# dotchen/LAV

Measured on AMD Instinct MI355X. Metric: frames/s full agent fwd (32k-pt LiDAR + 3 cams), higher is better.
Workload: dtype f32 (convolution contractions on the matrix cores with f32 accumulate at the error of an fp32 dot product, DESIGN 4.3: the layers on the split-operand kernel - BEV backbone, heads, crop stems, the brake net's mid-size layers - and ERFNet's persistent runs of pairs as two power-of-two-scaled fp16 pie

## Files before the change

### include/lav_amd.h

```cpp
#ifndef LAV_AMD_H
#define LAV_AMD_H

#include <stddef.h>
#include <stdint.h>

#ifdef __cplusplus
extern "C" {
#endif

#define LAV_ABI_VERSION 30

#define LAV_OK 0
#define LAV_EINVAL (-1)
#define LAV_EHIP (-2)
#define LAV_EWORKSPACE (-3)

int lav_abi_version(void);
const char *lav_last_error(void);
int lav_device_count(void);

int lav_profile_enable(int slots);
int lav_profile_reset(void);
int lav_profile_read(const char *kernel, double *total_ms, int *launches);

typedef struct lav_grid {
    float min_x, max_x, min_y, max_y;
    float ppm;
    int nx, ny;
} lav_grid;

typedef struct lav_pointnet {
    const float *w1, *b1, *w2, *b2;
    int num_input;
// ... 187 lines not shown

size_t lav_upconv_pointwise_packed_floats(int cin, int cout, int k);
int lav_upconv_pointwise_pack(int cin, int cout, int k, const float *h_weight, float *h_packed);
int lav_upconv_pointwise_parts(int batch, int cin, int cout, int ih, int iw, int k, int pad, int out_pad);
int lav_upconv_pointwise(int batch, int cin, int cout, int ih, int iw, int k, int pad, int out_pad, const float *x, const float *w_packed,
                         const float *scale, const float *shift, int relu_pre, int out_c_total, int out_c_offset, float *y,
                         float *amax_out, void *stream);

size_t lav_conv1d_pair_packed_weight_floats(int channels);
int lav_conv1d_pair_pack_weights(int channels, const float *h_weight, float *h_packed);
size_t lav_conv1d_pair_chain_workspace_bytes(int batch, int h);
size_t lav_conv1d_pair_chain_lds_bytes(int channels, int w, int d_b_max);
int lav_conv1d_pair_chain(int batch, int channels, int h, int w, int npairs, const int *d_a, const int *d_b, const int *residual,
                          const int *relu_post, const float *x, const float *const *wa_packed, const float *const *bias_a,
                          const float *const *wb_packed, const float *const *bias_b, const float *const *scale,
                          const float *const *shift, float *const *out, void *workspace, size_t workspace_bytes, void *stream);
int lav_conv1d_pair_chain_f16(int batch, int channels, int h, int w, int npairs, const int *d_a, const int *d_b, const int *residual,
                              const int *relu_post, const float *x, const float *const *wa_packed, const float *const *bias_a,
                              const float *const *wb_packed, const float *const *bias_b, const float *const *scale,
                              const float *const *shift, float *const *out, void *workspace, size_t workspace_bytes, void *stream);
int lav_conv1d_pair_chain_region(int row_offset, int clean_rows);
int lav_conv1d_pair_chain_status(const void *workspace, int *h_timeouts_launches2, void *stream);
size_t lav_conv1d_pair_lds_bytes(int channels, int w, int d_b);
int lav_conv1d_pair(int batch, int channels, int h, int w, int d_a, int d_b, const float *x, const float *wa_packed,
                    const float *bias_a, const float *wb_packed, const float *bias_b, const float *scale, const float *shift,
                    const float *residual, int relu_post, float *y, void *stream);

int lav_pool_affine(const float *x, int batch, int channels, int h, int w, const float *scale, const float *shift, int relu,
                    float *y, int out_c_total, int out_c_offset, void *stream);

int lav_pair_train_supported(int channels, int width);
size_t lav_pair_train_workspace_bytes(int batch, int channels, int h);
int lav_pair_train_forward(const float *x, const float *wa, const float *ba, const float *wb, const float *bb, int batch, int channels,
                           int h, int w, int dil, float *t, float *z, void *stream);
int lav_pair_train_backward(const float *x, const float *t, const float *dz, const float *wa, const float *wb, int batch, int channels,
                            int h, int w, int dil, float *dt, float *dx, float *dwa, float *dba, float *dwb, float *dbb, void *workspace,
                            size_t workspace_bytes, void *stream);

size_t lav_seg_xent_workspace_bytes(void);
int lav_seg_xent_forward(const float *logits, const long long *labels, int batch, int classes, long plane, float *loss, float *dlogits,
                         void *workspace, size_t workspace_bytes, void *stream);

int lav_seg_xent_up_forward(const float *logits, const void *labels, int label_bytes, int batch, int classes, int h, int w, int scale,
                            float *loss, float *dlogits, void *workspace, size_t workspace_bytes, void *stream);

#ifdef __cplusplus
// ... 4 lines not shown
```

### lav_amd/_lib.py

```python
from __future__ import annotations

import ctypes as C
import os

HERE = os.path.dirname(os.path.abspath(__file__))
LIB_PATH = os.environ.get("LAV_AMD_LIB") or os.path.join(HERE, "liblav_amd.so")

ABI_VERSION = 30
MAX_CAM = 4


class Grid(C.Structure):
    _fields_ = [("min_x", C.c_float), ("max_x", C.c_float), ("min_y", C.c_float), ("max_y", C.c_float),
                ("ppm", C.c_float), ("nx", C.c_int), ("ny", C.c_int)]


class PointNet(C.Structure):
    _fields_ = [("w1", C.c_void_p), ("b1", C.c_void_p), ("w2", C.c_void_p), ("b2", C.c_void_p),
                ("num_input", C.c_int), ("channels", C.c_int)]


class Camera(C.Structure):
    _fields_ = [("K", C.c_float * 9), ("l2w", C.c_float * 16), ("w2c", C.c_float * 16)]


class Conv(C.Structure):
    _fields_ = [(n, C.c_int) for n in (
        "batch", "in_c_total", "in_c_offset", "cin", "h", "w", "cout", "kh", "kw", "stride", "pad_h", "pad_w",
        "dil_h", "dil_w", "transposed", "out_pad", "out_c_total", "out_c_offset", "relu_pre", "relu_post", "sigmoid", "target_cus")] + [("pad_value", C.c_float), ("precision", C.c_int)]


# ... 42 lines not shown
    "lav_conv2d": (_I, [C.POINTER(Conv), _P, _P, _P, _P, _P, _P, _P, _P, _Z, _P]),
    "lav_conv_amax_count": (_I, [C.POINTER(Conv)]),
    "lav_conv2d_amax": (_I, [C.POINTER(Conv), _P, _P, _P, _P, _P, _P, _P, _P, _Z, _P, _I, _P, _P]),
    "lav_deconv_grouped": (_I, [_I, _I, _I, _I, _I, C.POINTER(_I), _I, _I, _I, _I, _P, _P, _P, _I, _P, _P]),
    "lav_crop_rotate": (_I, [_P, _I, _I, _I, _I, _P, _P, _I, _F, _I, _F, _F, _P, _P]),
    "lav_crop_rotate_indexed": (_I, [_P, _I, _P, _I, _I, _I, _P, _P, _I, _F, _I, _F, _F, _P, _P]),
    "lav_crop_rotate_backward": (_I, [_P, _I, _P, _I, _I, _I, _P, _P, _I, _F, _I, _F, _F, _P, _P]),
    "lav_pillar_decorate": (_I, [_P, C.POINTER(_I), _I, _I, _I, C.POINTER(Grid), _P, _P, _P, _P, _P, _P, _Z, _P]),
    "lav_scatter_max": (_I, [_P, _P, _I, _I, _I, _P, _P, _P]),
    "lav_scatter_max_backward": (_I, [_P, _P, _I, _I, _I, _P, _P]),
    "lav_conv1d_pair_packed_weight_floats": (_Z, [_I]),
    "lav_conv1d_pair_pack_weights": (_I, [_I, _P, _P]),
    "lav_upconv_pointwise_packed_floats": (_Z, [_I, _I, _I]),
    "lav_upconv_pointwise_pack": (_I, [_I, _I, _I, _P, _P]),
    "lav_upconv_pointwise_parts": (_I, [_I] * 8),
    "lav_upconv_pointwise": (_I, [_I] * 8 + [_P, _P, _P, _P, _I, _I, _I, _P, _P, _P]),
    "lav_conv1d_pair_chain_workspace_bytes": (_Z, [_I, _I]),
    "lav_conv1d_pair_chain_region": (_I, [_I, _I]),
    "lav_conv1d_pair_chain_lds_bytes": (_Z, [_I, _I, _I]),
    "lav_conv1d_pair_chain": (_I, [_I, _I, _I, _I, _I, C.POINTER(_I), C.POINTER(_I), C.POINTER(_I), C.POINTER(_I), _P] + [C.POINTER(_P)] * 7 + [_P, _Z, _P]),
    "lav_conv1d_pair_chain_f16": (_I, [_I, _I, _I, _I, _I, C.POINTER(_I), C.POINTER(_I), C.POINTER(_I), C.POINTER(_I), _P] + [C.POINTER(_P)] * 7 + [_P, _Z, _P]),
    "lav_conv1d_pair_chain_status": (_I, [_P, C.POINTER(_I), _P]),
    "lav_conv1d_pair_lds_bytes": (_Z, [_I, _I, _I]),
    "lav_conv1d_pair": (_I, [_I, _I, _I, _I, _I, _I, _P, _P, _P, _P, _P, _P, _P, _P, _I, _P, _P]),
    "lav_gru_seq_forward": (_I, [_P, _I, _P, _P, _P, _I, _I, _I, _P, _P, _P]),
    "lav_gru_seq_backward_workspace_bytes": (_Z, [_I, _I]),
    "lav_gru_seq_backward": (_I, [_P, _P, _P, _P, _P, _I, _I, _I, _P, _P, _P, _P, _Z, _P]),
    "lav_bn_train_workspace_bytes": (_Z, [_I]),
    "lav_bn_train_forward_mask": (_I, [_P, _P, _P, _P, _I, _I, C.c_long, _P, _P, C.c_double, _I, _P, _P, _P, _P, _P, _Z, _P]),
    "lav_bn_train_backward_mask": (_I, [_P, _P, _P, _P, _I, _I, C.c_long, _P, _P, _P, _I, _P, _P, _P, _P, _P, _P, _Z, _P]),
    "lav_pair_train_supported": (_I, [_I, _I]),
    "lav_pair_train_workspace_bytes": (_Z, [_I, _I, _I]),
    "lav_pair_train_forward": (_I, [_P, _P, _P, _P, _P, _I, _I, _I, _I, _I, _P, _P, _P]),
    "lav_pair_train_backward": (_I, [_P, _P, _P, _P, _P, _I, _I, _I, _I, _I, _P, _P, _P, _P, _P, _P, _P, _Z, _P]),
    "lav_seg_xent_workspace_bytes": (_Z, []),
    "lav_seg_xent_forward": (_I, [_P, _P, _I, _I, C.c_long, _P, _P, _P, _Z, _P]),
    "lav_seg_xent_up_forward": (_I, [_P, _P, _I, _I, _I, _I, _I, _I, _P, _P, _P, _Z, _P]),
    "lav_attn_train_workspace_bytes": (_Z, [_I, _I, _I, _I]),
    "lav_attn_train_forward": (_I, [_P, _I, _I, _I, _I, _P, _P, _P, _P, C.c_float, _P, _P, _P, _P, _P, _P]),
    "lav_attn_train_backward": (_I, [_P, _I, _I, _I, _I, _P, _P, _P, _P, C.c_float, _P, _P, _P, _P, _P, _P, _P, _P, _P, _Z, _P]),
    "lav_bn_train_forward": (_I, [_P, _P, _P, _I, _I, C.c_long, _P, _P, C.c_double, _I, _I, _P, _P, _P, _P, _Z, _P]),
    "lav_bn_train_backward": (_I, [_P, _P, _P, _I, _I, C.c_long, _P, _P, _P, _I, _I, _P, _P, _P, _P, _P, _Z, _P]),
    "lav_bn_train_amax_count": (_I, [_I, _I, C.c_long]),
    "lav_bn_train_forward_amax": (_I, [_P, _P, _P, _I, _I, C.c_long, _P, _P, C.c_double, _I, _I, _P, _P, _P, _P, _P, _Z, _P]),
    "lav_bn_train_backward_amax": (_I, [_P, _P, _P, _I, _I, C.c_long, _P, _P, _P, _I, _I, _P, _P, _P, _P, _P, _P, _Z, _P]),
    "lav_attn_pool": (_I, [_P, _I, _I, _I, _I, _P, _P, _P, _P, _P, _P]),
# ... 53 lines not shown
```

### lav_amd/build.py

```python
from __future__ import annotations

import os
import subprocess
import sys
import time

HERE = os.path.dirname(os.path.abspath(__file__))
REPO = os.path.dirname(HERE)
CSRC = os.path.join(HERE, "csrc")
LIB = os.path.join(HERE, "liblav_amd.so")
SOURCES = ["misc.hip", "pillar.hip", "paint.hip", "gru.hip", "gru_seq.hip", "conv.hip", "conv_f16.hip", "conv_pair.hip", "deconv.hip", "crop.hip", "frame.hip", "attn.hip", "bn_train.hip", "conv_wgrad.hip", "upconv.hip", "conv_pair_train.hip"]
EXTRA_FLAGS = {"pillar.hip": ["-ffp-contract=off"], "paint.hip": ["-ffp-contract=off"], "crop.hip": ["-ffp-contract=off"],
               "frame.hip": ["-ffp-contract=off"]}
FLAGS = ["--offload-arch=gfx950", "-O3", "-std=c++17", "-fPIC", "-Wall", "-Wno-unused-function", "-fno-slp-vectorize",
         "-I", os.path.join(REPO, "include"), "-I", CSRC]


def _hipcc() -> str:
    for c in (os.environ.get("HIPCC"), "/opt/rocm/bin/hipcc", "hipcc"):
        if c and (os.path.isabs(c) and os.path.exists(c) or not os.path.isabs(c)):
            return c
    raise RuntimeError("hipcc not found")


def needs_build() -> bool:
    if not os.path.exists(LIB):
        return True
    t = os.path.getmtime(LIB)
    deps = [os.path.join(CSRC, f) for f in os.listdir(CSRC)] + [os.path.join(REPO, "include", "lav_amd.h")]
    return any(os.path.getmtime(d) > t for d in deps)


def build(force: bool = False, verbose: bool = True) -> str:
    if not force and not needs_build():
# ... 28 lines not shown
```

### lav_amd/csrc/conv.hip

```cpp
#include <algorithm>
#include <cstdlib>
#include <cstring>
#include <vector>

#include "common.hpp"
#include "conv_f16.hpp"

namespace {
using namespace lav;
typedef float f32x16 __attribute__((ext_vector_type(16)));

constexpr int MAX_TAPS = 64;
constexpr int MAX_CLASSES = 16;
constexpr int CK = 16;
constexpr int TAP_GROUP = 9;
constexpr int NPOS_MAX = 40;

struct ConvArgs {
    const float *x, *w, *bias, *scale, *shift, *res;
    const int *n_valid;
    unsigned long long *trace;
    float *y;
    int in_c_total, in_c_offset, cin, H, W;
    int cout, out_c_total, out_c_offset, OH, OW;
// ... 824 lines not shown
}
}

extern "C" int lav_conv_out_hw(const lav_conv *c, int *oh, int *ow) {
    LAV_REQUIRE(c, "lav_conv_out_hw: null");
    Plan p;
    int rc = build_plan(*c, p);
    if (rc) return rc;
    if (oh) *oh = p.OH;
    if (ow) *ow = p.OW;
    return LAV_OK;
}

extern "C" size_t lav_conv_packed_weight_floats(const lav_conv *c) {
    if (!c) return 0;
    Plan p;
    if (build_plan(*c, p)) return 0;
    const int prec = resolve_precision(*c);
    size_t n = has_split_packing(prec) ? (p.wfloats + 3) / 4 * 4 + split_weight_bytes(p) / 4 : p.wfloats;
    if (prec == LAV_CONV_F16X3 && f16x3_layer(*c, p)) n += split_weight_bytes_f16(p) / 4 + 4;
    return n;
}

extern "C" int lav_conv_pack_weights(const lav_conv *c, const float *h_weight, float *h_packed) {
    LAV_REQUIRE(c && h_weight && h_packed, "lav_conv_pack_weights: null");
    Plan p;
    int rc = build_plan(*c, p);
    if (rc) return rc;
    memset(h_packed, 0, p.wfloats * sizeof(float));
    for (int cls = 0; cls < p.nclasses; ++cls) {
        float *dst = h_packed + p.woff[cls];
        const auto &t = p.taps[cls];
        parallel_for((int)t.size(), [&, dst](int ti_) {
            const size_t ti = (size_t)ti_;
            for (int ci = 0; ci < c->cin; ++ci)
                for (int co = 0; co < c->cout; ++co) {
                    const size_t src = c->transposed
                                           ? (((size_t)ci * c->cout + co) * c->kh + t[ti].ky) * c->kw + t[ti].kx
                                           : (((size_t)co * c->cin + ci) * c->kh + t[ti].ky) * c->kw + t[ti].kx;
                    dst[(size_t)(co / 32) * t.size() * p.cin_pad * 32 + ((ti * p.cin_pad + ci) / 8) * 256 + ((ci & 1) * 32 + co % 32) * 4 + (ci % 8) / 2] = h_weight[src];
                }
        });
    }
    if (has_split_packing(resolve_precision(*c)))
        split_pack_weights(*c, p, h_weight, reinterpret_cast<unsigned char *>(h_packed + (p.wfloats + 3) / 4 * 4));
    if (resolve_precision(*c) == LAV_CONV_F16X3 && f16x3_layer(*c, p))
// ... 339 lines not shown
```

### lav_amd/frame.py

```python
from __future__ import annotations

import math
import os
import time
from collections import deque

import numpy as np
import torch

from . import ops
from .model_inference import InferModel

GAP = 5
_COPY_STREAM = os.environ.get("LAV_COPY_STREAM", "0") == "1"
_DET_REPORT = os.environ.get("LAV_DET_REPORT", "1") != "0"
_POSE_BLOCK = os.environ.get("LAV_POSE_BLOCK", "1") != "0"
_BRAKE_AFTER = os.environ.get("LAV_BRAKE_AFTER", "in")
_BRAKE_SPLIT = os.environ.get("LAV_BRAKE_SPLIT", "wide")
if _BRAKE_SPLIT in ("0", "off", "none"):
    _BRAKE_SPLIT = ""
_DIAG_SKIP = set(filter(None, os.environ.get("LAV_DIAG_SKIP", "").split(",")))


def ego_box_mask(lidar: torch.Tensor) -> torch.Tensor:
# ... 458 lines not shown
                       crop_size=up.crop_size * 2, cmd=int(cmd_value), impl="steps")[0, -1, 0]
        self.plan_aborts += 1
        return plan

    @torch.no_grad()
    @_at_frame_precision
    def plan_deviation(self, out, cmd_value) -> float:
        up = self.infer_model.uniplanner
        with torch.cuda.stream(self.s_ego):
            self.s_ego.wait_stream(torch.cuda.current_stream())
            ego_cast = up.cast(out["ego_embd"], mode="ego")
            plan = up.plan(out["ego_embd"], self.b_nxp[None], cast_locs=ego_cast, pixels_per_meter=up.pixels_per_meter,
                           crop_size=up.crop_size * 2, cmd=int(cmd_value), impl="steps")[0, -1, 0]
            dev = (plan - out["ego_plan_locs"]).abs().max()
        torch.cuda.current_stream().wait_stream(self.s_ego)
        return float(dev)

    def health(self, cmd_value: int = 3) -> dict:
        torch.cuda.synchronize()
        up = self.infer_model.uniplanner
        diag = ops.gru_plan_diag(1, up.plan_gru.hidden_size, up.num_cmds, int(cmd_value), self.device, stream=self.s_ego)
        nonfinite, checks = (int(v) for v in self.d_health.cpu())
        chain_timeouts, chain_launches = ops.pair_chain_status(self.device, stream=self.s_cap)
        nonfinite += self.nonfinite_det_frames
        return dict(nonfinite_outputs=nonfinite, finite_checks=checks, plan_launches=diag["launches"], plan_aborts=diag["aborted_launches"],
                    pair_chain_launches=chain_launches, pair_chain_timeouts=chain_timeouts,
                    plans_recomputed=self.plan_aborts, decode_mismatches=self.decode_mismatches, overflow_ticks=self.overflow_ticks,
                    last_plan_launch=diag)

    @torch.no_grad()
    @_at_frame_precision
    def precapture(self, cmds=range(6), max_others=15):
        dev, P = self.device, self.P
        tick = torch.zeros((P, 4), dtype=torch.float32, device=dev)
        tick[:, 0] = torch.linspace(5.0, 60.0, P, device=dev); tick[:, 2] = -1.0
        rgb = lambda *shape: torch.zeros(shape, dtype=torch.float32, device=dev)
        args = (rgb(3, 3, 288, 256), rgb(1, 3, 288, 768), rgb(1, 3, 192, 480), np.zeros(2), 0.0, torch.zeros(2, device=dev))
        self.step(tick, *args, 3)
        self.step(tick, *args, 3)
        for cmd in cmds:
            with torch.cuda.stream(self.s_ego):
                self._replay(("ego", int(cmd)), self._g_ego, self.s_ego, int(cmd))
        if self.device_others:
            self._replay("others_cap", self._g_others_cap, self.s_cap)
        else:
            for n in range(1, max_others + 1):
                self._replay(("others", n), self._g_others, self.s_cap, n)
        torch.cuda.synchronize()
        self.reset()
# ... 4 lines not shown
```

### lav_amd/lidar.py

```python
from __future__ import annotations

import torch
from torch import nn
import torch.nn.functional as F

from . import _lib
from . import ops
from .ops import Amax, ConvLayer, GroupedDeconv, PointwiseUpconv
from .point_pillar import PointPillarNet

_NORM = dict(eps=1e-3, momentum=0.01)


def _refreshable(obj):
    if isinstance(obj, dict):
        for v in obj.values():
            yield from _refreshable(v)
    elif isinstance(obj, (list, tuple)):
        for v in obj:
            yield from _refreshable(v)
    elif hasattr(obj, "refresh"):
        yield obj


class _Engine(nn.Module):

    def _drop(self):
        object.__setattr__(self, "_eng", None)
        object.__setattr__(self, "_stale", False)

    def _mark_stale(self):
# ... 69 lines not shown
        eng = self._fresh(device) or dict(device=device)
        key = ("backbone", prec)
        if key in eng:
            return eng[key]
        def stage(seq):
            out = []
            for j in range(0, len(seq), 3):
                conv, bn = seq[j], seq[j + 2]
                out.append(ConvLayer(conv.weight, stride=conv.stride[0], padding=conv.padding, bn=_bn_tuple(bn),
                                     bn_eps=bn.eps, relu_pre=True, precision=prec, device=device))
            return out
        ups = []
        off = 0
        for seq in (self.upconv1, self.upconv2, self.upconv3):
            ct, bn = seq[0], seq[2]
            if prec == _lib.CONV_F16X3 and PointwiseUpconv.takes(ct):
                ups.append(PointwiseUpconv(ct, bn, relu_pre=True, out_c_total=self.out_channels, out_c_offset=off, device=device))
            else:
                ups.append(ConvLayer(ct.weight, stride=ct.stride[0], padding=ct.padding, transposed=True,
                                     output_padding=ct.output_padding[0], bn=_bn_tuple(bn), bn_eps=bn.eps, relu_pre=True,
                                     out_c_total=self.out_channels, out_c_offset=off, precision=prec, device=device))
            off += ct.weight.shape[1]
        eng[key] = dict(s1=stage(self.conv1), s2=stage(self.conv2), s3=stage(self.conv3), ups=ups, amax={}, f16=prec == _lib.CONV_F16X3)
        eng["tensor_ids"] = self._tensor_ids()
        object.__setattr__(self, "_eng", eng)
        return eng[key]

    def forward_train(self, x):
        from .train.hipnn import conv_relu_bn
        f1 = conv_relu_bn(self.conv1, x)
        f2 = conv_relu_bn(self.conv2, f1)
        f3 = conv_relu_bn(self.conv3, f2)
        return torch.cat([conv_relu_bn(self.upconv1, f1), conv_relu_bn(self.upconv2, f2), conv_relu_bn(self.upconv3, f3)], dim=1)

    def forward(self, x, out=None):
        if self.training:
            return self.forward_train(x)
        self._need_eval()
        e = self._engine(x.device)
        if not e["f16"]:
            feats = []
            for st in (e["s1"], e["s2"], e["s3"]):
                for layer in st:
                    x = layer(x)
                feats.append(x)
            oh, ow = e["ups"][0].out_hw(feats[0].shape[2], feats[0].shape[3])
            if out is None:
                out = torch.empty((x.shape[0], self.out_channels, oh, ow), dtype=torch.float32, device=x.device)
            for up, f in zip(e["ups"], feats):
                up(f, out=out)
            return out
        B = x.shape[0]
        key = ops.amax_key(x)
        ams = e["amax"].get(key)
        if ams is None:
            ams = e["amax"][key] = [Amax(x.device) for _ in range(len(e["s1"]) + len(e["s2"]) + len(e["s3"]) + 1)]
        stages = (e["s1"], e["s2"], e["s3"])
        feats, feat_am, am_prev, i = [], [], ops.amax_of(x), 0
        for si, st in enumerate(stages):
            for li, layer in enumerate(st):
                oh, ow = layer.out_hw(x.shape[2], x.shape[3])
                readers = ([st[li + 1]] if li + 1 < len(st) else ([stages[si + 1][0]] if si + 1 < len(stages) else [])) + \
                          ([e["ups"][si]] if li + 1 == len(st) else [])
                am = ams[i].reset() if any(r.uses_amax(B, oh, ow) for r in readers) else None
                x = layer(x, amax_in=am_prev, amax_out=am)
                am_prev, i = am, i + 1
            feats.append(x); feat_am.append(am_prev)
        oh, ow = e["ups"][0].out_hw(feats[0].shape[2], feats[0].shape[3])
        if out is None:
            out = torch.empty((B, self.out_channels, oh, ow), dtype=torch.float32, device=x.device)
        am_out = ams[-1].reset()
        for up, f, am in zip(e["ups"], feats, feat_am):
            up(f, out=out, amax_in=am, amax_out=am_out)
        return ops.tag_amax(out, am_out)


class Head(_Engine):
    def __init__(self, num_input, num_output, num_hidden=64, norm_cfg=None, output_activation=nn.Identity()):
        super().__init__()
        self.net = nn.Sequential(
            nn.Conv2d(num_input, num_hidden, 3, 1, 1, bias=False),
            nn.ReLU(inplace=True),
            nn.BatchNorm2d(num_hidden, **_NORM),
            nn.ConvTranspose2d(num_hidden, num_output, 3, 2, 1, 1),
        )
        self.output_activation = output_activation
        self._drop()

    @property
# ... 93 lines not shown
```

### lav_amd/ops.py

```python
from __future__ import annotations

import ctypes as C
import os as _os
import threading as _threading
from typing import Optional, Sequence

import numpy as np
import torch

from . import _lib
from ._lib import Camera, Conv, Grid, PointNet, check

_workspaces: dict = {}


def _stream() -> int:
    return torch.cuda.current_stream().cuda_stream


def _ptr(t: Optional[torch.Tensor]) -> Optional[int]:
    return None if t is None else t.data_ptr()


def _f32c(t: torch.Tensor, name: str) -> torch.Tensor:
# ... 743 lines not shown

    def __enter__(self):
        check(_lib.load().lav_conv1d_pair_chain_region(*self.args), "lav_conv1d_pair_chain_region")
        return self

    def __exit__(self, *exc):
        check(_lib.load().lav_conv1d_pair_chain_region(0, -1), "lav_conv1d_pair_chain_region")
        return False


def pair_chain_status(device, stream=None):
    st = stream if stream is not None else torch.cuda.current_stream()
    device = torch.device(device)
    if device.index is None:
        device = torch.device("cuda", torch.cuda.current_device())
    ws = _workspaces.get(("pair_chain", device, st.cuda_stream))
    if ws is None:
        return (0, 0)
    v = (C.c_int * 2)()
    check(_lib.load().lav_conv1d_pair_chain_status(_ptr(ws), v, st.cuda_stream), "lav_conv1d_pair_chain_status")
    return (int(v[0]), int(v[1]))


_CU_COUNT = {}


def _cu_count(device) -> int:
    idx = torch.device(device).index
    idx = torch.cuda.current_device() if idx is None else idx
    if idx not in _CU_COUNT:
        _CU_COUNT[idx] = torch.cuda.get_device_properties(idx).multi_processor_count
    return _CU_COUNT[idx]


train_work = {"crop_rotate_backward_bytes": 0, "crop_rotate_backward_calls": 0, "gru_seq_forward_flops": 0, "gru_seq_backward_flops": 0,
              "bn_train_fwd_bytes": 0, "bn_train_bwd_bytes": 0, "conv_wgrad_flops": 0}


class _CropRotateIndexed(torch.autograd.Function):

    @staticmethod
    def forward(ctx, features, map_index, locs, oris, ppm, crop, ox, oy):
        lib = _lib.load()
        features = _f32c(features, "features")
        locs, oris = _f32c(locs.detach().reshape(-1, 2), "locs"), _f32c(oris.detach().reshape(-1), "oris")
        if map_index.dtype != torch.int32 or not map_index.is_cuda:
# ... 218 lines not shown
```

Measured before the change: 508.0.

## Fuse BEV backbone stage conv3x3 layers into one persistent fp16-split run kernel

Adds a persistent kernel that runs a stage's sequence of identical 3x3 conv + ReLU + BatchNorm layers in one launch. Blocks own output rows and wait on per-row readiness words from the previous layer instead of relaunching. It applies to the BEV backbone stages s2 and s3 by default, cutting per-layer launch overhead and letting weight prefetch overlap across layers. In exchange it relies on inter-block spin-waiting with a timeout and NaN-fill fallback, and adds ping-pong intermediate buffers.

```diff
diff --git a/include/lav_amd.h b/include/lav_amd.h
--- a/include/lav_amd.h
+++ b/include/lav_amd.h
@@ -8,7 +8,7 @@
 extern "C" {
 #endif
 
-#define LAV_ABI_VERSION 30
+#define LAV_ABI_VERSION 31
 
 #define LAV_OK 0
 #define LAV_EINVAL (-1)
@@ -242,6 +242,15 @@
 int lav_conv1d_pair_chain_region(int row_offset, int clean_rows);
 int lav_conv1d_pair_chain_status(const void *workspace, int *h_timeouts_launches2, void *stream);
 size_t lav_conv1d_pair_lds_bytes(int channels, int w, int d_b);
+size_t lav_conv3x3_run_f16_workspace_bytes(int channels, int h, int w, int nlayers);
+size_t lav_conv3x3_run_f16_lds_bytes(int channels, int h, int w);
+size_t lav_conv3x3_run_f16_weight_bytes(int channels);
+int lav_conv3x3_run_f16_amax_count(int channels, int h, int w);
+long lav_conv_f16_weights_offset(const lav_conv *c);
+int lav_conv3x3_run_f16(int channels, int h, int w, int nlayers, const float *x, const void *const *w_f16, const float *const *scale,
+                        const float *const *shift, float *out, const float *amax_in, int amax_in_count, float *amax_out, void *workspace,
+                        size_t workspace_bytes, void *stream);
+int lav_conv3x3_run_f16_status(const void *workspace, int *h_timeouts_launches2, void *stream);
 int lav_conv1d_pair(int batch, int channels, int h, int w, int d_a, int d_b, const float *x, const float *wa_packed,
                     const float *bias_a, const float *wb_packed, const float *bias_b, const float *scale, const float *shift,
                     const float *residual, int relu_post, float *y, void *stream);
diff --git a/lav_amd/_lib.py b/lav_amd/_lib.py
--- a/lav_amd/_lib.py
+++ b/lav_amd/_lib.py
@@ -6,7 +6,7 @@
 HERE = os.path.dirname(os.path.abspath(__file__))
 LIB_PATH = os.environ.get("LAV_AMD_LIB") or os.path.join(HERE, "liblav_amd.so")
 
-ABI_VERSION = 30
+ABI_VERSION = 31
 MAX_CAM = 4
 
 
@@ -95,6 +95,13 @@
     "lav_conv1d_pair_chain_f16": (_I, [_I, _I, _I, _I, _I, C.POINTER(_I), C.POINTER(_I), C.POINTER(_I), C.POINTER(_I), _P] + [C.POINTER(_P)] * 7 + [_P, _Z, _P]),
     "lav_conv1d_pair_chain_status": (_I, [_P, C.POINTER(_I), _P]),
     "lav_conv1d_pair_lds_bytes": (_Z, [_I, _I, _I]),
+    "lav_conv3x3_run_f16_workspace_bytes": (_Z, [_I, _I, _I, _I]),
+    "lav_conv3x3_run_f16_lds_bytes": (_Z, [_I, _I, _I]),
+    "lav_conv3x3_run_f16_weight_bytes": (_Z, [_I]),
+    "lav_conv3x3_run_f16_amax_count": (_I, [_I, _I, _I]),
+    "lav_conv_f16_weights_offset": (C.c_long, [C.POINTER(Conv)]),
+    "lav_conv3x3_run_f16": (_I, [_I, _I, _I, _I, _P, C.POINTER(_P), C.POINTER(_P), C.POINTER(_P), _P, _P, _I, _P, _P, _Z, _P]),
+    "lav_conv3x3_run_f16_status": (_I, [_P, C.POINTER(_I), _P]),
     "lav_conv1d_pair": (_I, [_I, _I, _I, _I, _I, _I, _P, _P, _P, _P, _P, _P, _P, _P, _I, _P, _P]),
     "lav_gru_seq_forward": (_I, [_P, _I, _P, _P, _P, _I, _I, _I, _P, _P, _P]),
     "lav_gru_seq_backward_workspace_bytes": (_Z, [_I, _I]),
diff --git a/lav_amd/build.py b/lav_amd/build.py
--- a/lav_amd/build.py
+++ b/lav_amd/build.py
@@ -9,7 +9,7 @@
 REPO = os.path.dirname(HERE)
 CSRC = os.path.join(HERE, "csrc")
 LIB = os.path.join(HERE, "liblav_amd.so")
-SOURCES = ["misc.hip", "pillar.hip", "paint.hip", "gru.hip", "gru_seq.hip", "conv.hip", "conv_f16.hip", "conv_pair.hip", "deconv.hip", "crop.hip", "frame.hip", "attn.hip", "bn_train.hip", "conv_wgrad.hip", "upconv.hip", "conv_pair_train.hip"]
+SOURCES = ["misc.hip", "pillar.hip", "paint.hip", "gru.hip", "gru_seq.hip", "conv.hip", "conv_f16.hip", "conv_pair.hip", "conv_run.hip", "deconv.hip", "crop.hip", "frame.hip", "attn.hip", "bn_train.hip", "conv_wgrad.hip", "upconv.hip", "conv_pair_train.hip"]
 EXTRA_FLAGS = {"pillar.hip": ["-ffp-contract=off"], "paint.hip": ["-ffp-contract=off"], "crop.hip": ["-ffp-contract=off"],
                "frame.hip": ["-ffp-contract=off"]}
 FLAGS = ["--offload-arch=gfx950", "-O3", "-std=c++17", "-fPIC", "-Wall", "-Wno-unused-function", "-fno-slp-vectorize",
diff --git a/lav_amd/csrc/conv.hip b/lav_amd/csrc/conv.hip
--- a/lav_amd/csrc/conv.hip
+++ b/lav_amd/csrc/conv.hip
@@ -870,6 +870,14 @@
     return n;
 }
 
+extern "C" long lav_conv_f16_weights_offset(const lav_conv *c) {
+    if (!c) return -1;
+    Plan p;
+    if (build_plan(*c, p)) return -1;
+    if (resolve_precision(*c) != LAV_CONV_F16X3 || !f16x3_layer(*c, p)) return -1;
+    return (long)((p.wfloats + 3) / 4 * 4 + split_weight_bytes(p) / 4);
+}
+
 extern "C" int lav_conv_pack_weights(const lav_conv *c, const float *h_weight, float *h_packed) {
     LAV_REQUIRE(c && h_weight && h_packed, "lav_conv_pack_weights: null");
     Plan p;
diff --git a/lav_amd/csrc/conv_run.hip b/lav_amd/csrc/conv_run.hip
--- /dev/null
+++ b/lav_amd/csrc/conv_run.hip
@@ -0,0 +1,375 @@
+#include <cstdlib>
+#include <cstring>
+
+#include "common.hpp"
+
+namespace {
+using namespace lav;
+typedef float f32x16 __attribute__((ext_vector_type(16)));
+typedef unsigned u32x4 __attribute__((ext_vector_type(4)));
+typedef _Float16 run_f16x2 __attribute__((ext_vector_type(2)));
+typedef _Float16 run_f16x8 __attribute__((ext_vector_type(8)));
+typedef float run_f32x2 __attribute__((ext_vector_type(2)));
+
+constexpr int RUN_MAX = 8;
+constexpr int RUN_MAX_WG = 256;
+constexpr size_t RUN_ZERO_CAP = 16 + (size_t)RUN_MAX * RUN_MAX_WG * 8;
+constexpr size_t RUN_STICKY_OFF = RUN_ZERO_CAP;
+constexpr size_t RUN_MAPS_OFF = (RUN_STICKY_OFF + 16 + 255) / 256 * 256;
+constexpr int RUN_TAIL_LDS = 2 * 128 * 4 + 64;
+
+struct RunArgs {
+    const float *x;
+    float *out, *map[2];
+    const unsigned char *w[RUN_MAX];
+    const float *wscale[RUN_MAX], *scale[RUN_MAX], *shift[RUN_MAX];
+    const float *amax_in;
+    float *amax_out;
+    unsigned long long *words;
+    int *abort_word, *sticky;
+    long long spin_limit;
+    int amax_in_count, C, H, W, L, NS, data_bytes;
+};
+
+__device__ __forceinline__ void run_split2h(float u0, float u1, unsigned &q0, unsigned &q1) {
+    const run_f16x2 h0 = __builtin_convertvector(run_f32x2{u0, u1}, run_f16x2);
+    const run_f32x2 f0 = __builtin_convertvector(h0, run_f32x2);
+    const run_f16x2 h1 = __builtin_convertvector(run_f32x2{u0 - f0[0], u1 - f0[1]}, run_f16x2);
+    q0 = __builtin_bit_cast(unsigned, h0);
+    q1 = __builtin_bit_cast(unsigned, h1);
+}
+
+template <int NPB, int NCBW, int KS, int NTK>
+__global__ __launch_bounds__(512) void k_conv3x3_run_f16(RunArgs a) {
+    static_assert(NCBW * KS == 8, "eight waves");
+    extern __shared__ __attribute__((aligned(16))) unsigned char smem[];
+    const int tid = threadIdx.x, lane = tid & 63, l31 = lane & 31, half = lane >> 5;
+    const int wid = __builtin_amdgcn_readfirstlane(tid >> 6);
+    const int cbw = wid % NCBW, kp = wid / NCBW;
+    const int C = a.C, H = a.H, W = a.W, L = a.L, NS = a.NS;
+    const int y = blockIdx.x / NS, s = blockIdx.x - y * NS;
+    const int nchunk = C >> 4, G8 = C >> 3, WP = W + 2, nper = nchunk / KS;
+    const int cb = s * NCBW + cbw;
+    const long plane = (long)H * W;
+    const int piece = G8 * 3 * WP * 16;
+    float *s_red = reinterpret_cast<float *>(smem);
+    float *s_epi = reinterpret_cast<float *>(smem + a.data_bytes);
+    float *s_wmax = s_epi + 256;
+    float *s_m = s_wmax + 8;
+    int *s_abort = reinterpret_cast<int *>(s_m + 4);
+    if (tid == 0) *s_abort = 0;
+    if (blockIdx.x == 0 && tid == 0) atomicAdd(a.sticky + 1, 1);
+
+    u32x4 wr[9][2];
+    auto load_w = [&](const unsigned char *p, int t, u32x4 (&dst)[2]) {
+        dst[0] = *reinterpret_cast<const u32x4 *>(p + (long)t * nchunk * 2048);
+        dst[1] = *reinterpret_cast<const u32x4 *>(p + (long)t * nchunk * 2048 + 1024);
+    };
+    const long wlane = ((long)cb * 9 * nchunk + kp * nper) * 2048 + lane * 16;
+#pragma unroll
+    for (int t = 0; t < 9; ++t) load_w(a.w[0] + wlane, t, wr[t]);
+    float m_in = parts_absmax(a.amax_in, a.amax_in_count, lane);
+
+    int pxb[NPB];
+#pragma unroll
+    for (int pb = 0; pb < NPB; ++pb) pxb[pb] = min(pb * 32 + l31, W - 1);
+
+    for (int l = 0; l < L; ++l) {
+        const bool last = l + 1 == L;
+        const float *src = l == 0 ? a.x : a.map[(l - 1) & 1];
+        float *dst = last ? a.out : a.map[l & 1];
+        if (tid >= 64 && tid < 64 + C) {
+            s_epi[tid - 64] = a.scale[l][tid - 64];
+            s_epi[128 + tid - 64] = a.shift[l][tid - 64];
+        }
+        if (l > 0) {
+            if (wid == 0) {
+                const int rr = y - 1 + lane / NS, ss = lane % NS;
+                const bool need = lane < 3 * NS && rr >= 0 && rr < H;
+                const unsigned long long *wp = a.words + (long)(l - 1) * H * NS + (need ? rr * NS + ss : 0);
+                unsigned long long wv = (unsigned long long)l << 32;
+                long long spins = 0;
+                bool ok = false;
+                while (true) {
+                    if (need) wv = __hip_atomic_load(wp, __ATOMIC_RELAXED, __HIP_MEMORY_SCOPE_AGENT);
+                    ok = __all((int)(wv >> 32) == l);
+                    if (ok) break;
+                    ++spins;
+                    const bool timed_out = spins > a.spin_limit;
+                    const bool peer_gone = !timed_out && (spins & 63) == 0 && __hip_atomic_load(a.abort_word, __ATOMIC_RELAXED, __HIP_MEMORY_SCOPE_AGENT) != 0;
+                    if (timed_out || peer_gone) {
+                        if (lane == 0) {
+                            *s_abort = 1;
+                            if (timed_out) { atomicAdd(a.sticky, 1); __hip_atomic_store(a.abort_word, 1, __ATOMIC_RELAXED, __HIP_MEMORY_SCOPE_AGENT); }
+                        }
+                        break;
+                    }
+                    __builtin_amdgcn_s_sleep(1);
+                }
+                if (ok) {
+                    const float m = wave_finite_absmax(need ? finite_abs(__uint_as_float((unsigned)wv)) : 0.f);
+                    if (lane == 0) s_m[0] = m;
+                }
+            }
+            __syncthreads();
+            if (*(volatile int *)s_abort) {
+                const int nco = NCBW * 32;
+                for (int i = tid; i < nco * W; i += 512) a.out[(long)(s * nco + i / W) * plane + (long)y * W + (i % W)] = __uint_as_float(0x7fc00000u);
+                if (tid == 0 && a.amax_out) a.amax_out[blockIdx.x] = 0.f;
+                return;
+            }
+            m_in = s_m[0];
+        }
+        for (int i = tid; i < 2 * G8 * 3 * 2; i += 512) {
+            const int side = i & 1, q = i >> 1;
+            *reinterpret_cast<u32x4 *>(smem + ((long)q * WP + (side ? WP - 1 : 0)) * 16) = u32x4{0u, 0u, 0u, 0u};
+        }
+        const float sx = f16_scale_of(m_in), inv = 1.f / sx;
+        {
+            float v[NTK][16];
+            bool okr[NTK];
+            const int ntask = nchunk * 3 * W;
+#pragma unroll
+            for (int u = 0; u < NTK; ++u) {
+                const int task = tid + u * 512;
+                const int tk = min(task, ntask - 1);
+                const int q = tk / W, px = tk - q * W, c = q / 3, t = q - 3 * c;
+                const int yy = y + t - 1;
+                okr[u] = task < ntask && yy >= 0 && yy < H;
+                const float *sp = src + ((long)c * 16 * H + (okr[u] ? yy : y)) * W + px;
+#pragma unroll
+                for (int ch = 0; ch < 16; ++ch) v[u][ch] = __hip_atomic_load(sp + ch * plane, __ATOMIC_RELAXED, __HIP_MEMORY_SCOPE_AGENT);
+            }
+#pragma unroll
+            for (int u = 0; u < NTK; ++u) {
+                const int task = tid + u * 512;
+                if (task < ntask) {
+                    const int q = task / W, px = task - q * W, c = q / 3, t = q - 3 * c;
+#pragma unroll
+                    for (int h = 0; h < 2; ++h) {
+                        u32x4 q2[2];
+#pragma unroll
+                        for (int e = 0; e < 4; ++e) {
+                            unsigned p0, p1;
+                            const float x0 = okr[u] ? v[u][8 * h + 2 * e] : 0.f, x1 = okr[u] ? v[u][8 * h + 2 * e + 1] : 0.f;
+                            run_split2h(x0 * inv, x1 * inv, p0, p1);
+                            q2[0][e] = p0; q2[1][e] = p1;
+                        }
+                        const int entry = ((c * 2 + h) * 3 + t) * WP + px + 1;
+                        *reinterpret_cast<u32x4 *>(smem + entry * 16) = q2[0];
+                        *reinterpret_cast<u32x4 *>(smem + piece + entry * 16) = q2[1];
+                    }
+                }
+            }
+        }
+        __syncthreads();
+        float out_sx, out_sw;
+        {
+            int ex = 0, ew = 0;
+            (void)frexpf(sx, &ex);
+            (void)frexpf(*a.wscale[l], &ew);
+            const int et = ex + ew - 2;
+            out_sx = ldexpf(1.f, et >> 1); out_sw = ldexpf(1.f, et - (et >> 1));
+        }
+
+        f32x16 acc[NPB];
+#pragma unroll
+        for (int pb = 0; pb < NPB; ++pb)
+#pragma unroll
+            for (int r = 0; r < 16; ++r) acc[pb][r] = 0.f;
+        const unsigned char *w_this = a.w[l] + wlane, *w_next = a.w[last ? l : l + 1] + wlane;
+        for (int ci = 0; ci < nper; ++ci) {
+            const int ch = kp * nper + ci;
+            const unsigned char *w_refill = ci + 1 < nper ? w_this + (ci + 1) * 2048 : w_next;
+            const unsigned char *bin = smem + ((ch * 2 + half) * 3 * WP) * 16;
+#pragma unroll
+            for (int t = 0; t < 9; ++t) {
+                const int toff = ((t / 3) * WP + (t % 3)) * 16;
+#pragma unroll
+                for (int g0 = 0; g0 < NPB; g0 += 3) {
+                    constexpr int GMAX = 3;
+                    u32x4 b[GMAX][2];
+#pragma unroll
+                    for (int j = 0; j < GMAX; ++j)
+                        if (g0 + j < NPB) {
+                            b[j][0] = *reinterpret_cast<const u32x4 *>(bin + toff + pxb[g0 + j] * 16);
+                            b[j][1] = *reinterpret_cast<const u32x4 *>(bin + piece + toff + pxb[g0 + j] * 16);
+                        }
+#pragma unroll
+                    for (int j = 0; j < GMAX; ++j)
+                        if (g0 + j < NPB)
+                            acc[g0 + j] = __builtin_amdgcn_mfma_f32_32x32x16_f16(__builtin_bit_cast(run_f16x8, wr[t][1]), __builtin_bit_cast(run_f16x8, b[j][0]), acc[g0 + j], 0, 0, 0);
+#pragma unroll
+                    for (int j = 0; j < GMAX; ++j)
+                        if (g0 + j < NPB)
+                            acc[g0 + j] = __builtin_amdgcn_mfma_f32_32x32x16_f16(__builtin_bit_cast(run_f16x8, wr[t][0]), __builtin_bit_cast(run_f16x8, b[j][1]), acc[g0 + j], 0, 0, 0);
+#pragma unroll
+                    for (int j = 0; j < GMAX; ++j)
+                        if (g0 + j < NPB)
+                            acc[g0 + j] = __builtin_amdgcn_mfma_f32_32x32x16_f16(__builtin_bit_cast(run_f16x8, wr[t][0]), __builtin_bit_cast(run_f16x8, b[j][0]), acc[g0 + j], 0, 0, 0);
+                }
+                load_w(w_refill, t, wr[t]);
+            }
+        }
+        __syncthreads();
+#pragma unroll
+        for (int pb = 0; pb < NPB; ++pb) {
+            const int o = pb % KS;
+            if (kp != o) {
+                const int idx = kp < o ? kp : kp - 1;
+                float *d = s_red + ((long)((idx * NCBW + cbw) * NPB + pb) * 16) * 64 + lane;
+#pragma unroll
+                for (int r = 0; r < 16; ++r) d[r * 64] = acc[pb][r];
+            }
+        }
+        __syncthreads();
+        float lm = 0.f;
+#pragma unroll
+        for (int pb = 0; pb < NPB; ++pb) {
+            const int o = pb % KS;
+            if (kp == o) {
+                f32x16 tot;
+#pragma unroll
+                for (int r = 0; r < 16; ++r) tot[r] = 0.f;
+#pragma nounroll
+                for (int k = 0; k < KS; ++k) {
+                    if (k == o) {
+#pragma unroll
+                        for (int r = 0; r < 16; ++r) tot[r] += acc[pb][r];
+                    } else {
+                        const int idx = k < o ? k : k - 1;
+                        const float *d = s_red + ((long)((idx * NCBW + cbw) * NPB + pb) * 16) * 64 + lane;
+#pragma unroll
+                        for (int r = 0; r < 16; ++r) tot[r] += d[r * 64];
+                    }
+                }
+                const int px = pb * 32 + l31;
+                float *yo = dst + (long)y * W + px;
+#pragma unroll
+                for (int r = 0; r < 16; ++r) {
+                    const int co = cb * 32 + (r & 3) + 8 * (r >> 2) + 4 * half;
+                    float vv = tot[r] * out_sx * out_sw;
+                    vv = vv > 0.f ? vv : 0.f;
+                    vv = fmaf(vv, s_epi[co], s_epi[128 + co]);
+                    if (px < W) {
+                        if (last) yo[co * plane] = vv;
+                        else __hip_atomic_store(yo + co * plane, vv, __ATOMIC_RELAXED, __HIP_MEMORY_SCOPE_AGENT);
+                        lm = fmaxf(lm, finite_abs(vv));
+                    }
+                }
+            }
+        }
+        lm = wave_finite_absmax(lm);
+        if (lane == 0) s_wmax[wid] = lm;
+        asm volatile("s_waitcnt vmcnt(0)" ::: "memory");
+        __syncthreads();
+        if (tid == 0) {
+            float m = 0.f;
+#pragma unroll
+            for (int i = 0; i < 8; ++i) m = fmaxf(m, s_wmax[i]);
+            if (last) {
+                if (a.amax_out) a.amax_out[blockIdx.x] = m;
+            } else {
+                __hip_atomic_store(a.words + (long)l * H * NS + blockIdx.x, ((unsigned long long)(l + 1) << 32) | __float_as_uint(m), __ATOMIC_RELAXED,
+                                   __HIP_MEMORY_SCOPE_AGENT);
+            }
+        }
+    }
+}
+
+struct RunConfig { int NS, NCBW, KS, NPB, NTK; size_t data_bytes, map_bytes; };
+
+bool run_config(int channels, int h, int w, RunConfig &c) {
+    if ((channels != 64 && channels != 128) || h < 1 || w < 1 || w > 160) return false;
+    if (channels == 64) c.NS = 1;
+    else c.NS = h * 4 <= RUN_MAX_WG ? 4 : 2;
+    if (h * c.NS > RUN_MAX_WG) return false;
+    c.NCBW = channels / 32 / c.NS; c.KS = 8 / c.NCBW;
+    if (c.NCBW * c.KS != 8 || (channels / 16) % c.KS) return false;
+    c.NPB = w <= 64 ? 2 : w <= 96 ? 3 : 5;
+    const int ntask = channels / 16 * 3 * w;
+    c.NTK = ntask <= 1024 ? 2 : ntask <= 2048 ? 4 : 0;
+    if (!c.NTK) return false;
+    const size_t rows = (size_t)2 * (channels / 8) * 3 * (w + 2) * 16, red = (size_t)(c.KS - 1) * c.NCBW * c.NPB * 4096;
+    c.data_bytes = (std::max(rows, red) + 255) / 256 * 256;
+    if (c.data_bytes + RUN_TAIL_LDS > 160 * 1024) return false;
+    c.map_bytes = ((size_t)channels * h * w * sizeof(float) + 255) / 256 * 256;
+    return true;
+}
+}
+
+extern "C" size_t lav_conv3x3_run_f16_workspace_bytes(int channels, int h, int w, int nlayers) {
+    RunConfig c;
+    if (nlayers < 1 || nlayers > RUN_MAX || !run_config(channels, h, w, c)) return 0;
+    return RUN_MAPS_OFF + 2 * c.map_bytes;
+}
+
+extern "C" size_t lav_conv3x3_run_f16_lds_bytes(int channels, int h, int w) {
+    RunConfig c;
+    if (!run_config(channels, h, w, c)) return 0;
+    return c.data_bytes + RUN_TAIL_LDS;
+}
+
+extern "C" int lav_conv3x3_run_f16_amax_count(int channels, int h, int w) {
+    RunConfig c;
+    return run_config(channels, h, w, c) ? h * c.NS : 0;
+}
+
+extern "C" size_t lav_conv3x3_run_f16_weight_bytes(int channels) {
+    if (channels < 32 || channels % 32) return 0;
+    return (size_t)9 * (channels / 32) * (channels / 16) * 2 * 1024;
+}
+
+extern "C" int lav_conv3x3_run_f16(int channels, int h, int w, int nlayers, const float *x, const void *const *w_f16, const float *const *scale,
+                                   const float *const *shift, float *out, const float *amax_in, int amax_in_count, float *amax_out, void *workspace,
+                                   size_t workspace_bytes, void *stream) {
+    RunConfig c;
+    LAV_REQUIRE(nlayers >= 1 && nlayers <= RUN_MAX, "lav_conv3x3_run_f16: 1..%d layers", RUN_MAX);
+    LAV_REQUIRE(run_config(channels, h, w, c), "lav_conv3x3_run_f16: %d channels on %d x %d is not served (lav_conv3x3_run_f16_workspace_bytes returns 0)", channels, h, w);
+    LAV_REQUIRE(x && w_f16 && scale && shift && out && amax_in && amax_in_count >= 1, "lav_conv3x3_run_f16: null argument (the first layer's scale comes from amax_in)");
+    LAV_REQUIRE(workspace && workspace_bytes >= RUN_MAPS_OFF + 2 * c.map_bytes, "lav_conv3x3_run_f16: workspace too small");
+    RunArgs a;
+    char *ws = static_cast<char *>(workspace);
+    const size_t wbytes = lav_conv3x3_run_f16_weight_bytes(channels);
+    for (int i = 0; i < RUN_MAX; ++i) {
+        const int j = i < nlayers ? i : nlayers - 1;
+        LAV_REQUIRE(w_f16[j] && scale[j] && shift[j], "lav_conv3x3_run_f16: null argument of layer %d", j);
+        a.w[i] = static_cast<const unsigned char *>(w_f16[j]);
+        a.wscale[i] = reinterpret_cast<const float *>(a.w[i] + wbytes);
+        a.scale[i] = scale[j]; a.shift[i] = shift[j];
+    }
+    a.x = x; a.out = out;
+    a.map[0] = reinterpret_cast<float *>(ws + RUN_MAPS_OFF); a.map[1] = reinterpret_cast<float *>(ws + RUN_MAPS_OFF + c.map_bytes);
+    a.amax_in = amax_in; a.amax_in_count = amax_in_count; a.amax_out = amax_out;
+    a.abort_word = reinterpret_cast<int *>(ws); a.words = reinterpret_cast<unsigned long long *>(ws + 16);
+    a.sticky = reinterpret_cast<int *>(ws + RUN_STICKY_OFF);
+    const char *lim = getenv("LAV_CHAIN_SPIN_LIMIT");
+    a.spin_limit = lim ? std::max(0ll, atoll(lim)) : (1ll << 21);
+    a.C = channels; a.H = h; a.W = w; a.L = nlayers; a.NS = c.NS; a.data_bytes = (int)c.data_bytes;
+    hipStream_t st = static_cast<hipStream_t>(stream);
+    const int nwg = h * c.NS;
+    LAV_HIP(hipMemsetAsync(ws, 0, (16 + (size_t)(nlayers - 1) * nwg * 8 + 15) / 16 * 16, st));
+    const size_t lds = c.data_bytes + RUN_TAIL_LDS;
+    const int tok = timer_begin("conv3x3_run", st);
+    bool done = false;
+#define LAV_RUN_CASE(NPB_, NCBW_, KS_, NTK_) if (!done && c.NPB == NPB_ && c.NCBW == NCBW_ && c.KS == KS_ && c.NTK == NTK_) { \
+        static bool attr = false; \
+        if (!attr) { LAV_HIP(hipFuncSetAttribute(reinterpret_cast<const void *>(&k_conv3x3_run_f16<NPB_, NCBW_, KS_, NTK_>), hipFuncAttributeMaxDynamicSharedMemorySize, 160 * 1024)); attr = true; } \
+        hipLaunchKernelGGL((k_conv3x3_run_f16<NPB_, NCBW_, KS_, NTK_>), dim3(nwg), dim3(512), lds, st, a); \
+        done = true; }
+    LAV_RUN_CASE(5, 2, 4, 4) LAV_RUN_CASE(3, 2, 4, 4) LAV_RUN_CASE(3, 2, 4, 2) LAV_RUN_CASE(2, 2, 4, 4) LAV_RUN_CASE(2, 2, 4, 2)
+    LAV_RUN_CASE(2, 1, 8, 4) LAV_RUN_CASE(2, 1, 8, 2) LAV_RUN_CASE(3, 1, 8, 4)
+#undef LAV_RUN_CASE
+    timer_end(tok, st);
+    LAV_REQUIRE(done, "lav_conv3x3_run_f16: tile %d x %d / %d / %d not built", c.NPB, c.NCBW, c.KS, c.NTK);
+    LAV_LAUNCH_CHECK();
+    return LAV_OK;
+}
+
+extern "C" int lav_conv3x3_run_f16_status(const void *workspace, int *h_timeouts_launches2, void *stream) {
+    LAV_REQUIRE(workspace && h_timeouts_launches2, "lav_conv3x3_run_f16_status: bad argument");
+    hipStream_t st = static_cast<hipStream_t>(stream);
+    LAV_HIP(hipMemcpyAsync(h_timeouts_launches2, static_cast<const char *>(workspace) + RUN_STICKY_OFF, 2 * sizeof(int), hipMemcpyDeviceToHost, st));
+    LAV_HIP(hipStreamSynchronize(st));
+    return LAV_OK;
+}
diff --git a/lav_amd/frame.py b/lav_amd/frame.py
--- a/lav_amd/frame.py
+++ b/lav_amd/frame.py
@@ -504,9 +504,11 @@
         diag = ops.gru_plan_diag(1, up.plan_gru.hidden_size, up.num_cmds, int(cmd_value), self.device, stream=self.s_ego)
         nonfinite, checks = (int(v) for v in self.d_health.cpu())
         chain_timeouts, chain_launches = ops.pair_chain_status(self.device, stream=self.s_cap)
+        run_timeouts, run_launches = ops.bev_run_status(self.device, stream=self.s_cap)
         nonfinite += self.nonfinite_det_frames
         return dict(nonfinite_outputs=nonfinite, finite_checks=checks, plan_launches=diag["launches"], plan_aborts=diag["aborted_launches"],
-                    pair_chain_launches=chain_launches, pair_chain_timeouts=chain_timeouts,
+                    pair_chain_launches=chain_launches + run_launches, pair_chain_timeouts=chain_timeouts + run_timeouts,
+                    bev_run_launches=run_launches, bev_run_timeouts=run_timeouts,
                     plans_recomputed=self.plan_aborts, decode_mismatches=self.decode_mismatches, overflow_ticks=self.overflow_ticks,
                     last_plan_launch=diag)
 
diff --git a/lav_amd/lidar.py b/lav_amd/lidar.py
--- a/lav_amd/lidar.py
+++ b/lav_amd/lidar.py
@@ -6,7 +6,7 @@
 
 from . import _lib
 from . import ops
-from .ops import Amax, ConvLayer, GroupedDeconv, PointwiseUpconv
+from .ops import Amax, ConvLayer, ConvRun, GroupedDeconv, PointwiseUpconv
 from .point_pillar import PointPillarNet
 
 _NORM = dict(eps=1e-3, momentum=0.01)
@@ -122,6 +122,8 @@
                                      out_c_total=self.out_channels, out_c_offset=off, precision=prec, device=device))
             off += ct.weight.shape[1]
         eng[key] = dict(s1=stage(self.conv1), s2=stage(self.conv2), s3=stage(self.conv3), ups=ups, amax={}, f16=prec == _lib.CONV_F16X3)
+        want = ops.bev_run_stages() if prec == _lib.CONV_F16X3 else ()
+        eng[key]["runs"] = [ConvRun(eng[key][s][1:]) if s in want and len(eng[key][s]) > 2 else None for s in ("s1", "s2", "s3")]
         eng["tensor_ids"] = self._tensor_ids()
         object.__setattr__(self, "_eng", eng)
         return eng[key]
@@ -158,13 +160,18 @@
         stages = (e["s1"], e["s2"], e["s3"])
         feats, feat_am, am_prev, i = [], [], ops.amax_of(x), 0
         for si, st in enumerate(stages):
-            for li, layer in enumerate(st):
+            run, li = e["runs"][si], 0
+            while li < len(st):
+                layer = st[li]
                 oh, ow = layer.out_hw(x.shape[2], x.shape[3])
-                readers = ([st[li + 1]] if li + 1 < len(st) else ([stages[si + 1][0]] if si + 1 < len(stages) else [])) + \
-                          ([e["ups"][si]] if li + 1 == len(st) else [])
-                am = ams[i].reset() if any(r.uses_amax(B, oh, ow) for r in readers) else None
-                x = layer(x, amax_in=am_prev, amax_out=am)
-                am_prev, i = am, i + 1
+                runs_next = run is not None and run.takes(B, oh, ow)
+                n = len(st) - 1 if runs_next and li == 1 else 1
+                nxt = li + n
+                readers = ([run if runs_next and nxt == 1 else st[nxt]] if nxt < len(st) else ([stages[si + 1][0]] if si + 1 < len(stages) else [])) + \
+                          ([e["ups"][si]] if nxt == len(st) else [])
+                am = ams[i + n - 1].reset() if any(r.uses_amax(B, oh, ow) for r in readers) else None
+                x = (run if n > 1 else layer)(x, amax_in=am_prev, amax_out=am)
+                am_prev, i, li = am, i + n, nxt
             feats.append(x); feat_am.append(am_prev)
         oh, ow = e["ups"][0].out_hw(feats[0].shape[2], feats[0].shape[3])
         if out is None:
diff --git a/lav_amd/ops.py b/lav_amd/ops.py
--- a/lav_amd/ops.py
+++ b/lav_amd/ops.py
@@ -789,6 +789,84 @@
     return (int(v[0]), int(v[1]))
 
 
+def bev_run_stages():
+    v = _os.environ.get("LAV_BEV_RUN", BEV_RUN_DEFAULT).strip().lower()
+    if v in ("0", "", "off", "none"):
+        return frozenset()
+    if v in ("1", "on", "all"):
+        return frozenset(("s1", "s2", "s3"))
+    return frozenset(s for s in v.split(",") if s in ("s1", "s2", "s3"))
+
+
+BEV_RUN_DEFAULT = "s2,s3"
+
+
+class ConvRun:
+
+    def __init__(self, layers):
+        lib = _lib.load()
+        layers = list(layers)
+        l0 = layers[0]
+        for l in layers:
+            d = l.desc
+            if not (d.precision == _lib.CONV_F16X3 and (d.kh, d.kw, d.stride, d.pad_h, d.pad_w, d.dil_h, d.dil_w) == (3, 3, 1, 1, 1, 1, 1)
+                    and not d.transposed and l.cin == l.cout == l0.cin and l.in_c_total == l.cin and l.out_c_total == l.cout
+                    and l.bias is None and l.scale is not None and d.relu_pre and not d.relu_post and not d.sigmoid and d.pad_value == 0.0):
+                raise RuntimeError("ConvRun: layers must be identical conv3x3 / ReLU / BatchNorm layers packed for LAV_CONV_F16X3")
+        self.layers, self.ch = layers, l0.cin
+        probe = Conv.from_buffer_copy(l0.desc)
+        probe.h, probe.w = 64, 64
+        self._woff = int(lib.lav_conv_f16_weights_offset(C.byref(probe)))
+        if self._woff < 0 or len(layers) > 8:
+            raise RuntimeError("ConvRun: at most 8 layers with fp16 packed weights")
+        n = len(layers)
+        self._n = n
+
+    def takes(self, B: int, h: int, w: int) -> bool:
+        return B == 1 and _lib.load().lav_conv3x3_run_f16_workspace_bytes(self.ch, h, w, self._n) > 0
+
+    def uses_amax(self, B: int, h: int, w: int) -> bool:
+        return self.takes(B, h, w)
+
+    def __call__(self, x: torch.Tensor, out: Optional[torch.Tensor] = None, amax_in: Optional["Amax"] = None,
+                 amax_out: Optional["Amax"] = None) -> torch.Tensor:
+        lib = _lib.load()
+        x = _f32c(x, "x")
+        B, ch, h, w = x.shape
+        if ch != self.ch or not self.takes(B, h, w):
+            raise RuntimeError(f"ConvRun: input {tuple(x.shape)} is not served (lav_conv3x3_run_f16_workspace_bytes)")
+        if out is None:
+            out = torch.empty_like(x)
+        n = self._n
+        ws = _workspace(("conv_run", id(self), ch, h, w), lib.lav_conv3x3_run_f16_workspace_bytes(ch, h, w, n), x.device)
+        if amax_in is not None and amax_in.count > 0:
+            a_in, n_in = amax_in.buf, amax_in.count
+        else:
+            a_in = _workspace(("conv_run_amax", id(self)), 512 * 4, x.device).view(torch.float32)
+            n_in = 512
+            check(lib.lav_absmax_parts(_ptr(x), x.numel(), _ptr(a_in), _stream()), "lav_absmax_parts")
+        a_out = amax_out.take(lib.lav_conv3x3_run_f16_amax_count(ch, h, w)) if amax_out is not None else None
+        pa = lambda ts: (C.c_void_p * n)(*[t if isinstance(t, int) else t.data_ptr() for t in ts])
+        check(lib.lav_conv3x3_run_f16(ch, h, w, n, _ptr(x), pa([l.w.data_ptr() + 4 * self._woff for l in self.layers]),
+                                      pa([l.scale for l in self.layers]), pa([l.shift for l in self.layers]), _ptr(out), _ptr(a_in), n_in,
+                                      _ptr(a_out), _ptr(ws), ws.numel(), _stream()), "lav_conv3x3_run_f16")
+        return out
+
+
+def bev_run_status(device, stream=None):
+    st = stream if stream is not None else torch.cuda.current_stream()
+    device = torch.device(device)
+    if device.index is None:
+        device = torch.device("cuda", torch.cuda.current_device())
+    tot = [0, 0]
+    for (key, dev, s), ws in list(_workspaces.items()):
+        if isinstance(key, tuple) and key and key[0] == "conv_run" and dev == device and s == st.cuda_stream:
+            v = (C.c_int * 2)()
+            check(_lib.load().lav_conv3x3_run_f16_status(_ptr(ws), v, st.cuda_stream), "lav_conv3x3_run_f16_status")
+            tot[0] += int(v[0]); tot[1] += int(v[1])
+    return tuple(tot)
+
+
 _CU_COUNT = {}
 
 
```

After: 525.8 (median of 6 runs). 3.5% higher.
